# imdea-software/legosnark

Measured on AMD Instinct MI355X. Metric: alt_bn128 G1 MSM point-scalar pairs/s at n=2^20, higher is better.
Workload: dtype u32 limbs (254-bit Montgomery integers)

## Files before the change

### legosnark_amd/csrc/curves.h

```cpp
#pragma once
#include "ec.h"
#include "fp29.h"
#include "fp29x2.h"
#include "quad29.h"

namespace lsa {

struct CurveG1 {
    using Field = Fq;
    using Base = AffPacked;
    using Acc = XYZZ29;
    static constexpr bool GLV = true;
    static __device__ __forceinline__ Acc inf() { return Acc::inf(); }
    template <bool ENDO = true>
    static __device__ __forceinline__ Acc madd(const Acc &a, const Base &b, bool negate, bool endo) {
        return g1_madd_packed<ENDO>(a, b, negate, endo);
    }
    static constexpr bool HEAD = true;
    static __device__ __forceinline__ bool head_ok(const Base &b0, const Base &b1) { return !packed_is_inf(b0) && !packed_is_inf(b1); }
    template <bool ENDO = true>
    static __device__ __forceinline__ Acc madd_head(const Base &b0, bool neg0, bool endo0, const Base &b1, bool neg1, bool endo1) {
        return g1_madd_head<ENDO>(b0, neg0, endo0, b1, neg1, endo1);
    }
    static __device__ __forceinline__ Acc add(const Acc &a, const Acc &b) { return xyzz29_add(a, b); }
    static __device__ __forceinline__ Acc dbl(const Acc &a) { return xyzz29_dbl(a); }
    static __device__ __forceinline__ Jac<Fq> to_jac(const Acc &a) { return xyzz29_to_jac(a); }
    static __device__ __forceinline__ Acc from_jac(const Jac<Fq> &p) {
        if (p.Z.is_zero()) return Acc::inf();
        F29 z = F29::from_mont256(p.Z), zz = sqr(z);
        return {F29::from_mont256(p.X), F29::from_mont256(p.Y), zz, mul(zz, z)};
    }
    static __device__ __forceinline__ Base from_affine(const Aff<Fq> &a) {
        Base r;
        if (a.is_inf()) {
#pragma unroll
            for (int i = 0; i < 8; i++) { r.x[i] = 0; r.y[i] = 0; }
        } else {
            F29::from_mont256(a.x).canonical().pack256(r.x);
            F29::from_mont256(a.y).canonical().pack256(r.y);
        }
        return r;
    }
};
struct CurveG2 {
    using Field = Fq2;
    using Base = AffPackedG2;
    using Acc = XYZZ29x2;
    static constexpr bool GLV = false;
    static __device__ __forceinline__ Acc inf() { return Acc::inf(); }
    static constexpr bool HEAD = false;
    template <bool ENDO = true>
    static __device__ __forceinline__ Acc madd(const Acc &a, const Base &b, bool negate, bool ) {
        Aff29x2 q = unpack_affine(b);
        if (q.is_inf()) return a;
        if (negate) q.y = sub_k<1>(F29x2::zero(), q.y);
        return g2_madd(a, q);
    }
    static __device__ __forceinline__ Acc add(const Acc &a, const Acc &b) { return g2_add(a, b); }
    static __device__ __forceinline__ Acc dbl(const Acc &a) { return g2_dbl(a); }
    static __device__ __forceinline__ Jac<Fq2> to_jac(const Acc &a) { return g2_to_jac(a); }
    static __device__ __forceinline__ Acc from_jac(const Jac<Fq2> &p) {
        if (p.Z.is_zero()) return Acc::inf();
        F29x2 z = f29x2_from_mont256(p.Z), zz = sqr<2>(z);
        return {f29x2_from_mont256(p.X), f29x2_from_mont256(p.Y), zz, mul<2>(zz, z)};
    }
    static __device__ __forceinline__ Base from_affine(const Aff<Fq2> &a) { return pack_affine_g2(a); }
};
template <class F> struct CurveOf;
template <> struct CurveOf<Fq> { using type = CurveG1; };
template <> struct CurveOf<Fq2> { using type = CurveG2; };


}
```

### legosnark_amd/csrc/fp29.h

```cpp
#pragma once
#include "ec.h"

namespace lsa {

LSA_HD uint32_t lsa_mask(uint32_t m) {
#if defined(__HIP_DEVICE_COMPILE__)
    asm volatile("" : "+v"(m));
#endif
    return m;
}

struct F29 {
    static constexpr int W = 29;
    static constexpr uint32_t MASK = (1u << 29) - 1;
    static constexpr uint32_t PINV = 0x04866389u;
    static constexpr uint32_t PINV_POS = 0x1b799c77u;
    uint32_t l[9];

    static LSA_HD uint32_t p(int i) {
        constexpr uint32_t P29[9] = {0x187cfd47u, 0x010460b6u, 0x1c72a34fu, 0x02d522d0u, 0x1585d978u,
                                     0x02db40c0u, 0x00a6e141u, 0x0e5c2634u, 0x0030644eu};
        return P29[i];
    }
    static LSA_HD F29 from_limbs(const uint32_t (&c)[9]) {
        F29 r;
#pragma unroll
        for (int i = 0; i < 9; i++) r.l[i] = c[i];
        return r;
    }
    static LSA_HD F29 zero() {
        F29 r;
#pragma unroll
        for (int i = 0; i < 9; i++) r.l[i] = 0;
        return r;
    }
    static LSA_HD F29 one() {
        constexpr uint32_t C[9] = {0x157ccc21u, 0x141c2758u, 0x185230d3u, 0x014c0419u, 0x0aa36fb9u,
                                   0x1d4240ceu, 0x11d54c07u, 0x052ac7a8u, 0x000dc836u};
        return from_limbs(C);
    }
    LSA_HD bool limbs_zero() const {
        uint32_t o = 0;
#pragma unroll
        for (int i = 0; i < 9; i++) o |= l[i];
        return o == 0;
    }

    LSA_HD F29 norm() const {
        F29 r;
        int32_t c = 0;
#pragma unroll
        for (int i = 0; i < 8; i++) {
            int32_t v = (int32_t)l[i] + c;
            r.l[i] = (uint32_t)v & MASK;
            c = v >> 29;
        }
        r.l[8] = (uint32_t)((int32_t)l[8] + c);
        return r;
    }

    friend LSA_HD F29 add_lazy(const F29 &a, const F29 &b) {
        F29 r;
#pragma unroll
        for (int i = 0; i < 9; i++) r.l[i] = a.l[i] + b.l[i];
        return r;
    }
    template <int K>
    friend LSA_HD F29 sub_k(const F29 &a, const F29 &b);

    static LSA_HD F29 redc_cols(uint64_t (&col)[17]) {
        uint64_t carry = 0;
        F29 r;
#pragma unroll
        for (int k = 0; k < 9; k++) {
            uint64_t acc = col[k] + carry;
            const uint32_t m = ((uint32_t)acc * PINV) & MASK;
            acc += (uint64_t)m * p(0);
            carry = acc >> 29;
#pragma unroll
            for (int j = 1; j < 9; j++) col[k + j] += (uint64_t)m * p(j);
        }
#pragma unroll
        for (int k = 9; k < 17; k++) {
            const uint64_t acc = col[k] + carry;
            r.l[k - 9] = (uint32_t)acc & MASK;
            carry = acc >> 29;
        }
        r.l[8] = (uint32_t)carry;
        return r;
    }
    friend LSA_HD F29 mul(const F29 &a, const F29 &b) {
#if defined(LSA_FP29_COLS)
        {
            uint64_t col[17];
#pragma unroll
            for (int k = 0; k < 17; k++) col[k] = 0;
#pragma unroll
            for (int i = 0; i < 9; i++)
#pragma unroll
                for (int j = 0; j < 9; j++) col[i + j] += (uint64_t)a.l[i] * b.l[j];
            return redc_cols(col);
        }
#endif
        uint64_t acc = 0;
        uint32_t m[9];
        F29 r;
#pragma unroll
        for (int k = 0; k < 9; k++) {
#pragma unroll
            for (int i = 0; i <= k; i++) acc += (uint64_t)a.l[i] * b.l[k - i];
#pragma unroll
            for (int i = 0; i < k; i++) acc += (uint64_t)m[i] * p(k - i);
            m[k] = ((uint32_t)acc * PINV) & MASK;
            acc += (uint64_t)m[k] * p(0);
            acc >>= 29;
        }
#pragma unroll
        for (int k = 9; k < 17; k++) {
#pragma unroll
            for (int i = k - 8; i < 9; i++) acc += (uint64_t)a.l[i] * b.l[k - i];
#pragma unroll
            for (int i = k - 8; i < 9; i++) acc += (uint64_t)m[i] * p(k - i);
            r.l[k - 9] = (uint32_t)acc & MASK;
            acc >>= 29;
        }
        r.l[8] = (uint32_t)acc;
        return r;
    }
    friend LSA_HD F29 sqr(const F29 &a) {
        uint32_t d[9];
#pragma unroll
        for (int i = 0; i < 9; i++) d[i] = a.l[i] << 1;
#if defined(LSA_FP29_COLS)
        {
            uint64_t col[17];
#pragma unroll
            for (int k = 0; k < 17; k++) col[k] = 0;
#pragma unroll
            for (int i = 0; i < 9; i++) {
                col[2 * i] += (uint64_t)a.l[i] * a.l[i];
#pragma unroll
                for (int j = i + 1; j < 9; j++) col[i + j] += (uint64_t)a.l[i] * d[j];
            }
            return redc_cols(col);
        }
#endif
        uint64_t acc = 0;
        uint32_t m[9];
        F29 r;
#pragma unroll
        for (int k = 0; k < 17; k++) {
#pragma unroll
            for (int i = 0; i < 9; i++) {
// ... 88 lines not shown
                acc += (uint64_t)a1.l[i] * b1.l[k - i];
                acc += (uint64_t)a2.l[i] * b2.l[k - i];
                acc += (uint64_t)a3.l[i] * b3.l[k - i];
            }
#pragma unroll
            for (int i = k - 8; i < 9; i++) acc += (uint64_t)m[i] * p(k - i);
            r.l[k - 9] = (uint32_t)acc & MASK;
            acc >>= 29;
        }
        r.l[8] = (uint32_t)acc;
        return r;
    }
    friend LSA_HD F29 lin2(const F29 &u, int cu, const F29 &v, int cv, int K) {
        F29 r;
        int64_t c = 0;
#pragma unroll
        for (int i = 0; i < 9; i++) {
#if defined(__HIP_DEVICE_COMPILE__)
            int64_t t = c;
            asm("v_mad_i64_i32 %0, vcc, %1, %2, %0" : "+v"(t) : "v"(K), "v"((int32_t)p(i)) : "vcc");
            asm("v_mad_i64_i32 %0, vcc, %1, %2, %0" : "+v"(t) : "v"(cu), "v"((int32_t)u.l[i]) : "vcc");
            asm("v_mad_i64_i32 %0, vcc, %1, %2, %0" : "+v"(t) : "v"(cv), "v"((int32_t)v.l[i]) : "vcc");
#else
            const int64_t t = (int64_t)cu * (int64_t)u.l[i] + (int64_t)cv * (int64_t)v.l[i] + (int64_t)K * (int64_t)p(i) + c;
#endif
            if (i < 8) { r.l[i] = (uint32_t)t & MASK; c = t >> 29; }
            else r.l[i] = (uint32_t)t;
        }
        return r;
    }

    LSA_HD bool is_zero_mod_p() const {
        uint32_t k = (l[0] * PINV_POS) & MASK;
        if (k >= 16) return false;
        uint64_t c = 0;
        bool eq = true;
#pragma unroll
        for (int i = 0; i < 9; i++) {
            c += (uint64_t)k * p(i);
            uint32_t want = (i < 8) ? ((uint32_t)c & MASK) : (uint32_t)c;
            eq = eq && (want == l[i]);
            c >>= 29;
        }
        return eq;
    }

    LSA_HD F29 canonical() const {
        F29 t = *this;
#pragma unroll
        for (int s = 3; s >= 0; s--) {
            F29 d;
            int32_t c = 0;
            uint64_t pc = 0;
#pragma unroll
            for (int i = 0; i < 9; i++) {
                pc += (uint64_t)p(i) << s;
                uint32_t pl = (i < 8) ? ((uint32_t)pc & MASK) : (uint32_t)pc;
                pc >>= 29;
                int32_t v = (int32_t)t.l[i] - (int32_t)pl + c;
                if (i < 8) { d.l[i] = (uint32_t)v & MASK; c = v >> 29; }
                else d.l[i] = (uint32_t)v;
            }
            bool neg = ((int32_t)d.l[8]) < 0;
#pragma unroll
            for (int i = 0; i < 9; i++) t.l[i] = neg ? t.l[i] : d.l[i];
        }
        return t;
    }

    static LSA_HD F29 unpack256(const uint32_t w[8]) {
        F29 r;
#pragma unroll
        for (int i = 0; i < 9; i++) {
            const int bit = 29 * i, j = bit >> 5, s = bit & 31;
            uint64_t two = (uint64_t)w[j] | ((uint64_t)(j + 1 < 8 ? w[j + 1] : 0) << 32);
            r.l[i] = (uint32_t)(two >> s) & MASK;
        }
        return r;
    }
    LSA_HD void pack256(uint32_t w[8]) const {
#pragma unroll
        for (int j = 0; j < 8; j++) w[j] = 0;
#pragma unroll
        for (int i = 0; i < 9; i++) {
            const int bit = 29 * i, j = bit >> 5, s = bit & 31;
            uint64_t v = (uint64_t)l[i] << s;
            w[j] |= (uint32_t)v;
            if (j + 1 < 8) w[j + 1] |= (uint32_t)(v >> 32);
        }
    }
    static LSA_HD F29 from_mont256(const Fq &v) {
        constexpr uint32_t C[9] = {0x13349ca1u, 0x1a5d84a8u, 0x0a3e5cacu, 0x100249e0u, 0x12b951e8u,
                                   0x0e92d304u, 0x14cb95b3u, 0x041b9d3du, 0x00058003u};
        return mul(unpack256(v.l), from_limbs(C));
    }
    LSA_HD Fq to_mont256() const {
        constexpr uint32_t D[9] = {0x058f0d9du, 0x1aea1c6eu, 0x11c2cf74u, 0x11d651ebu, 0x1462c0a7u,
                                   0x11b7bc3cu, 0x1cbd99bau, 0x183340fbu, 0x000e0a77u};
        F29 t = mul(*this, from_limbs(D)).canonical();
        Fq r;
        t.pack256(r.l);
        return r;
    }
};

template <int K>
LSA_HD F29 sub_k(const F29 &a, const F29 &b) {
    F29 r;
    uint64_t pc = 0;
    int32_t c = 0;
#pragma unroll
    for (int i = 0; i < 9; i++) {
        pc += (uint64_t)F29::p(i) * (uint32_t)K;
        uint32_t kp = (i < 8) ? ((uint32_t)pc & F29::MASK) : (uint32_t)pc;
        pc >>= 29;
        int32_t v = (int32_t)a.l[i] + (int32_t)kp - (int32_t)b.l[i] + c;
        if (i < 8) { r.l[i] = (uint32_t)v & F29::MASK; c = v >> 29; }
        else r.l[i] = (uint32_t)v;
    }
    return r;
}

template <int K>
LSA_HD F29 sub_k_signed(const F29 &s, const F29 &b, uint32_t m) {
    F29 r;
    uint64_t pc = 0;
    const uint32_t m29 = m & F29::MASK;
    int32_t c = (int32_t)(m & 1u);
#pragma unroll
    for (int i = 0; i < 9; i++) {
        pc += (uint64_t)F29::p(i) * (uint32_t)K;
        uint32_t kp = (i < 8) ? ((uint32_t)pc & F29::MASK) : (uint32_t)pc;
        pc >>= 29;
        int32_t v = (int32_t)(s.l[i] ^ (i < 8 ? m29 : m)) + (int32_t)kp - (int32_t)b.l[i] + c;
        if (i < 8) { r.l[i] = (uint32_t)v & F29::MASK; c = v >> 29; }
        else r.l[i] = (uint32_t)v;
    }
    return r;
}

template <int K>
LSA_HD F29 sub_loose(const F29 &a, const F29 &b) {
    F29 r;
    uint64_t pc = 0;
#pragma unroll
    for (int i = 0; i < 9; i++) {
        pc += (uint64_t)F29::p(i) * (uint32_t)K;
        const uint32_t kp = (i < 8) ? ((uint32_t)pc & F29::MASK) : (uint32_t)pc;
        pc >>= 29;
        const uint32_t c = (i == 0) ? kp + (1u << 29) : (i < 8) ? kp + F29::MASK : kp - 1u;
        r.l[i] = a.l[i] + c - b.l[i];
    }
    return r;
}

struct Aff29 {
    F29 x, y;
    LSA_HD bool is_inf() const { return x.limbs_zero() && y.limbs_zero(); }
};
struct AffPacked {
    uint32_t x[8], y[8];
};
struct XYZZ29 {
    F29 X, Y, ZZ, ZZZ;
    LSA_HD bool is_inf() const { return ZZ.limbs_zero(); }
    static LSA_HD XYZZ29 inf() { return {F29::zero(), F29::zero(), F29::zero(), F29::zero()}; }
};

LSA_HD Aff29 unpack_affine(const AffPacked &q) { return {F29::unpack256(q.x), F29::unpack256(q.y)}; }

LSA_HD XYZZ29 xyzz29_dbl_affine(const Aff29 &b) {
    F29 U = add_lazy(b.y, b.y);
    F29 V = sqr(U);
    F29 W = mul(U, V);
    F29 S = mul(b.x, V);
    F29 xx = sqr(b.x);
    F29 M = add_lazy(add_lazy(xx, xx), xx).norm();
    F29 X3 = sub_k<4>(sqr(M), add_lazy(S, S));
    F29 Y3 = dot2(M, sub_k<8>(S, X3), W, sub_k<1>(F29::zero(), b.y));
    return {X3, Y3, V, W};
}

LSA_HD XYZZ29 xyzz29_dbl(const XYZZ29 &a) {
    if (a.is_inf()) return a;
    F29 U = add_lazy(a.Y, a.Y);
    F29 V = sqr(U);
    F29 W = mul(U, V);
    F29 S = mul(a.X, V);
    F29 xx = sqr(a.X);
    F29 M = add_lazy(add_lazy(xx, xx), xx).norm();
    F29 X3 = sub_k<4>(sqr(M), add_lazy(S, S));
    F29 Y3 = dot2(M, sub_k<8>(S, X3), W, sub_k<4>(F29::zero(), a.Y));
    return {X3, Y3, mul(V, a.ZZ), mul(W, a.ZZZ)};
}

LSA_HD XYZZ29 xyzz29_madd(const XYZZ29 &a, const Aff29 &b) {
    if (b.is_inf()) return a;
    if (a.is_inf()) return {b.x, b.y, F29::one(), F29::one()};
    F29 U2 = mul(b.x, a.ZZ);
    F29 S2 = mul(b.y, a.ZZZ);
    F29 Pd = sub_k<8>(U2, a.X);
    F29 R = sub_k<4>(S2, a.Y);
    if (Pd.is_zero_mod_p()) {
        if (R.is_zero_mod_p()) return xyzz29_dbl_affine(b);
        return XYZZ29::inf();
    }
    F29 PP = sqr(Pd);
    F29 PPP = mul(Pd, PP);
    F29 Q = mul(a.X, PP);
    F29 X3 = sub_k<6>(sqr(R), add_lazy(PPP, add_lazy(Q, Q)));
    F29 Y3 = dot2(R, sub_k<8>(Q, X3), sub_k<4>(F29::zero(), a.Y), PPP);
    return {X3, Y3, mul(a.ZZ, PP), mul(a.ZZZ, PPP)};
}

LSA_HD XYZZ29 xyzz29_madd_rare(const XYZZ29 &a, const Aff29 &b, uint32_t m, const F29 &R) {
    Aff29 q = b;
    if (m) q.y = sub_k<1>(F29::zero(), b.y);
    if (a.is_inf()) return {q.x, q.y, F29::one(), F29::one()};
    if (R.is_zero_mod_p()) return xyzz29_dbl_affine(q);
    return XYZZ29::inf();
}
LSA_HD XYZZ29 xyzz29_madd_signed(const XYZZ29 &a, const Aff29 &b, uint32_t m) {
    F29 U2 = mul(b.x, a.ZZ);
    F29 S2 = mul(b.y, a.ZZZ);
    F29 Pd = sub_k<8>(U2, a.X);
    F29 R = sub_k_signed<6>(S2, a.Y, m);
    if (Pd.is_zero_mod_p()) return xyzz29_madd_rare(a, b, m, R);
    F29 PP = sqr(Pd);
    F29 PPP = mul(Pd, PP);
    F29 Q = mul(a.X, PP);
    F29 X3 = sub_k<6>(sqr(R), add_lazy(PPP, add_lazy(Q, Q)));
    F29 Y3 = dot2(R, sub_loose<10>(Q, X3), sub_loose<6>(F29::zero(), a.Y), PPP);
    return {X3, Y3, mul(a.ZZ, PP), mul(a.ZZZ, PPP)};
}

LSA_HD XYZZ29 xyzz29_add_affine(const Aff29 &a, const Aff29 &b, uint32_t m) {
    F29 Pd = sub_k<2>(b.x, a.x);
    F29 R = sub_k_signed<2>(b.y, a.y, m);
    if (Pd.is_zero_mod_p()) {
        if (!R.is_zero_mod_p()) return XYZZ29::inf();
        Aff29 q = b;
        if (m) q.y = sub_k<1>(F29::zero(), b.y);
        return xyzz29_dbl_affine(q);
    }
    F29 PP = sqr(Pd);
    F29 PPP = mul(Pd, PP);
    F29 Q = mul(a.x, PP);
    F29 X3 = sub_k<6>(sqr(R), add_lazy(PPP, add_lazy(Q, Q)));
    F29 Y3 = dot2(R, sub_loose<10>(Q, X3), sub_loose<3>(F29::zero(), a.y), PPP);
    return {X3, Y3, PP, PPP};
}

LSA_HD XYZZ29 xyzz29_add(const XYZZ29 &a, const XYZZ29 &b) {
    if (b.is_inf()) return a;
    if (a.is_inf()) return b;
    F29 U1 = mul(a.X, b.ZZ);
    F29 U2 = mul(b.X, a.ZZ);
    F29 S1 = mul(a.Y, b.ZZZ);
    F29 S2 = mul(b.Y, a.ZZZ);
    F29 Pd = sub_k<2>(U2, U1);
    F29 R = sub_k<2>(S2, S1);
    if (Pd.is_zero_mod_p()) {
        if (R.is_zero_mod_p()) return xyzz29_dbl(a);
        return XYZZ29::inf();
    }
    F29 PP = sqr(Pd);
    F29 PPP = mul(Pd, PP);
    F29 Q = mul(U1, PP);
    F29 X3 = sub_k<6>(sqr(R), add_lazy(PPP, add_lazy(Q, Q)));
    F29 Y3 = dot2(R, sub_k<8>(Q, X3), sub_k<2>(F29::zero(), S1), PPP);
    return {X3, Y3, mul(mul(a.ZZ, b.ZZ), PP), mul(mul(a.ZZZ, b.ZZZ), PPP)};
}

LSA_HD bool packed_is_inf(const AffPacked &q) {
    if ((q.x[0] | q.y[0]) != 0) return false;
    uint32_t o = 0;
#pragma unroll
    for (int i = 1; i < 8; i++) o |= q.x[i] | q.y[i];
    return o == 0;
}
template <bool ENDO>
LSA_HD Aff29 g1_unpack_base(const AffPacked &b, bool endo) {
    Aff29 q = unpack_affine(b);
    if (ENDO && endo) {
        constexpr uint32_t BETA29[9] = {0x0a337995u, 0x158d1d23u, 0x189c9b98u, 0x12fa4e45u, 0x185faadcu,
                                        0x0176f16du, 0x0eed93bau, 0x14291140u, 0x000c0afeu};
        q.x = mul(q.x, F29::from_limbs(BETA29));
    }
    return q;
}
template <bool ENDO>
LSA_HD XYZZ29 g1_madd_packed(const XYZZ29 &a, const AffPacked &b, bool negate, bool endo) {
    if (packed_is_inf(b)) return a;
    return xyzz29_madd_signed(a, g1_unpack_base<ENDO>(b, endo), lsa_mask(negate ? ~0u : 0u));
}
template <bool ENDO>
LSA_HD XYZZ29 g1_madd_head(const AffPacked &b0, bool neg0, bool endo0, const AffPacked &b1, bool neg1, bool endo1) {
    Aff29 q0 = g1_unpack_base<ENDO>(b0, endo0);
    if (neg0) q0.y = sub_k<1>(F29::zero(), q0.y);
    return xyzz29_add_affine(q0, g1_unpack_base<ENDO>(b1, endo1), lsa_mask(neg1 ? ~0u : 0u));
}

LSA_HD XYZZ29 xyzz29_neg(const XYZZ29 &a) {
    if (a.is_inf()) return a;
    return {a.X, sub_k<4>(F29::zero(), a.Y), a.ZZ, a.ZZZ};
}

LSA_HD Jac<Fq> xyzz29_to_jac(const XYZZ29 &a) {
    if (a.is_inf()) return Jac<Fq>::inf();
    F29 Xj = mul(a.X, sqr(a.ZZ));
    F29 Yj = mul(a.Y, sqr(a.ZZZ));
    return {Xj.to_mont256(), Yj.to_mont256(), a.ZZZ.to_mont256()};
}

}
```

### legosnark_amd/csrc/msm.hip

```cpp
#include <hip/hip_runtime.h>
#include <stdint.h>
#include <stdio.h>
#include <stdlib.h>
#include <string.h>
#include <algorithm>
#include <type_traits>
#include <vector>

#include "curves.h"
#include "fp29x2l.h"
#include "fs29.h"
#include "glv.h"
#include "msm.h"
#include "msm_plan.h"

namespace lsa {


template <class F, int K>
__global__ __launch_bounds__(256) void k_normalize(const Jac<F> *__restrict__ in, Aff<F> *__restrict__ out, size_t n) {
    size_t t = (size_t)blockIdx.x * blockDim.x + threadIdx.x;
    size_t base = t * K;
    if (base >= n) return;
    F prod[K];
// ... 709 lines not shown
            perm[bin_start[bin] + lcnt[bin] + rank[j]] = g;
        }
    }
}

typedef uint32_t u32x4 __attribute__((ext_vector_type(4)));
template <class B> struct RawBase {
    static_assert(sizeof(B) % 16 == 0, "packed bases are whole 16-byte vectors");
    u32x4 q[sizeof(B) / 16];
};
template <class B>
__device__ __forceinline__ RawBase<B> load_base16(const B *__restrict__ p) {
    const u32x4 *src = reinterpret_cast<const u32x4 *>(p);
    RawBase<B> r;
#pragma unroll
    for (int i = 0; i < (int)(sizeof(B) / 16); i++) r.q[i] = src[i];
    return r;
}
template <class B>
__device__ __forceinline__ B packed_base(RawBase<B> r) {
    B b;
    uint32_t *dst = reinterpret_cast<uint32_t *>(&b);
#pragma unroll
    for (int i = 0; i < (int)(sizeof(B) / 16); i++) {
        asm("" : "+v"(r.q[i]));
        dst[4 * i] = r.q[i].x; dst[4 * i + 1] = r.q[i].y; dst[4 * i + 2] = r.q[i].z; dst[4 * i + 3] = r.q[i].w;
    }
    return b;
}
template <class C> struct RotatedLoads { static constexpr bool value = true; };
template <> struct RotatedLoads<CurveG2> { static constexpr bool value = false; };
template <class C, uint32_t ACC_SPLIT, bool ROTATED = RotatedLoads<C>::value>
__device__ __forceinline__ void accumulate_body(const typename C::Base *__restrict__ bases, const uint32_t *__restrict__ entries,
                                                const uint32_t *__restrict__ offs, const uint32_t *__restrict__ hist,
                                                const uint32_t *__restrict__ perm, const uint32_t *__restrict__ nperm,
                                                typename C::Acc *__restrict__ buckets) {
    uint32_t t = blockIdx.x * blockDim.x + threadIdx.x;
    if (t >= *nperm * ACC_SPLIT) return;
    const uint32_t g = perm[t / ACC_SPLIT], part = t % ACC_SPLIT;
    const uint32_t cnt = hist[g];
    const uint32_t *e = entries + offs[g];
    constexpr bool ENDO = ACC_SPLIT != 1;
    typename C::Acc acc = C::inf();
    if constexpr (!ROTATED) {
        if (part < cnt) {
            uint32_t v = e[part];
            typename C::Base cur = bases[v & 0x3fffffffu];
            static_assert(!C::HEAD || ROTATED, "the affine + affine head is written for the rotated loop only");
            for (uint32_t j = part; j < cnt; j += ACC_SPLIT) {
                uint32_t vn = v;
                typename C::Base nxt = cur;
                if (j + ACC_SPLIT < cnt) { vn = e[j + ACC_SPLIT]; nxt = bases[vn & 0x3fffffffu]; }
                acc = C::template madd<ENDO>(acc, cur, (v >> 31) != 0, ((v >> 30) & 1) != 0);
                v = vn;
                cur = nxt;
            }
        }
    } else if (part < cnt) {
        const uint32_t last = part + (cnt - 1 - part) / ACC_SPLIT * ACC_SPLIT;
        auto word = [&](uint32_t k) { return e[k < last ? k : last]; };
        auto base = [&](uint32_t w) { return load_base16(bases + (w & 0x3fffffffu)); };
        uint32_t j = part;
        uint32_t v = word(j), vn = word(j + ACC_SPLIT);
        RawBase<typename C::Base> cur;
        if constexpr (C::HEAD) {
            const uint32_t v2 = word(j + 2 * ACC_SPLIT), v3 = word(j + 3 * ACC_SPLIT);
            const RawBase<typename C::Base> r0 = base(v), r1 = base(vn), r2 = base(v2);
            const typename C::Base b0 = packed_base(r0), b1 = packed_base(r1);
            cur = r0;
            if (j + ACC_SPLIT < cnt && C::head_ok(b0, b1)) {
                acc = C::template madd_head<ENDO>(b0, (v >> 31) != 0, ((v >> 30) & 1) != 0, b1, (vn >> 31) != 0, ((vn >> 30) & 1) != 0);
                j += 2 * ACC_SPLIT;
                v = v2;
                vn = v3;
                cur = r2;
            }
        } else {
            cur = base(v);
        }
        for (; j < cnt; j += ACC_SPLIT) {
            const uint32_t vnn = word(j + 2 * ACC_SPLIT);
            const RawBase<typename C::Base> nxt = base(vn);
            acc = C::template madd<ENDO>(acc, packed_base(cur), (v >> 31) != 0, ((v >> 30) & 1) != 0);
            v = vn;
            vn = vnn;
            cur = nxt;
        }
    }
    buckets[(size_t)g * ACC_SPLIT + part] = acc;
}
template <class C, uint32_t ACC_SPLIT>
__global__ __launch_bounds__(256) void k_accumulate(const typename C::Base *__restrict__ bases, const uint32_t *__restrict__ entries,
                                                    const uint32_t *__restrict__ offs, const uint32_t *__restrict__ hist,
                                                    const uint32_t *__restrict__ perm, const uint32_t *__restrict__ nperm,
                                                    typename C::Acc *__restrict__ buckets) {
    accumulate_body<C, ACC_SPLIT>(bases, entries, offs, hist, perm, nperm, buckets);
}
__global__ __launch_bounds__(256) __attribute__((amdgpu_waves_per_eu(2, 2))) void k_accumulate_g2_occ2(
    const CurveG2::Base *__restrict__ bases, const uint32_t *__restrict__ entries, const uint32_t *__restrict__ offs,
    const uint32_t *__restrict__ hist, const uint32_t *__restrict__ perm, const uint32_t *__restrict__ nperm, CurveG2::Acc *__restrict__ buckets) {
    accumulate_body<CurveG2, 1u>(bases, entries, offs, hist, perm, nperm, buckets);
}

__global__ __launch_bounds__(256) void k_accumulate_g2_pair(const AffPackedG2 *__restrict__ bases, const uint32_t *__restrict__ entries,
                                                            const uint32_t *__restrict__ offs, const uint32_t *__restrict__ hist,
                                                            const uint32_t *__restrict__ perm, const uint32_t *__restrict__ nperm,
                                                            XYZZ29x2 *__restrict__ buckets) {
    const uint32_t t = blockIdx.x * blockDim.x + threadIdx.x, pr = t >> 1, part = t & 1;
    if (pr >= *nperm) return;
    const uint32_t g = perm[pr];
    const uint32_t cnt = hist[g];
    const uint32_t *e = entries + offs[g];
    struct Half { uint32_t x[8], y[8]; };
    auto fetch = [&](uint32_t v) {
        const AffPackedG2 &b = bases[v & 0x3fffffffu];
        Half h;
#pragma unroll
        for (int i = 0; i < 8; i++) { h.x[i] = b.w[part][i]; h.y[i] = b.w[2 + part][i]; }
        return h;
    };
    XyzzE<F29h> acc = XyzzE<F29h>::inf();
    uint32_t v = e[0];
    Half cur = fetch(v);
    for (uint32_t j = 0; j < cnt; j++) {
        uint32_t vn = v;
        Half nxt = cur;
        if (j + 1 < cnt) { vn = e[j + 1]; nxt = fetch(vn); }
        AffE<F29h> q = {{F29::unpack256(cur.x)}, {F29::unpack256(cur.y)}};
        if (!q.is_inf()) {
            if (v >> 31) q.y = sub_k<1>(F29h::zero(), q.y);
            acc = g2_madd(acc, q);
        }
        v = vn;
        cur = nxt;
    }
    F29 *o = reinterpret_cast<F29 *>(&buckets[g]);
    o[part] = acc.X.v;
    o[2 + part] = acc.Y.v;
    o[4 + part] = acc.ZZ.v;
    o[6 + part] = acc.ZZZ.v;
}

template <class A>
__device__ __forceinline__ A shfl_down_acc(const A &p, unsigned delta) {
    A r;
    constexpr int NW = sizeof(A) / 4;
    const uint32_t *src = reinterpret_cast<const uint32_t *>(&p);
    uint32_t *dst = reinterpret_cast<uint32_t *>(&r);
#pragma unroll
    for (int i = 0; i < NW; i++) dst[i] = __shfl_down(src[i], delta, 64);
    return r;
}

template <class C>
__device__ __forceinline__ typename C::Acc wave_sum(typename C::Acc v, unsigned lane) {
    for (unsigned d = 32; d >= 1; d >>= 1) {
        typename C::Acc t = shfl_down_acc(v, d);
        if (lane + d < 64) v = C::add(v, t);
    }
    return v;
}

__global__ __launch_bounds__(256) void k_heavy_plan(const uint32_t *__restrict__ hist, const uint32_t *__restrict__ heavy_list,
                                                    const uint32_t *__restrict__ heavy_count, uint32_t *__restrict__ chunk_off) {
    __shared__ uint32_t lds[4];
    __shared__ uint32_t s_chunk;
    const uint32_t nh = *heavy_count;
    uint32_t carry = 0;
    for (uint32_t base = 0; base < nh; base += 256) {
        uint32_t h = base + threadIdx.x;
        uint32_t tot;
        (void)block_exclusive_scan_256(h < nh ? hist[heavy_list[h]] : 0, lds, &tot);
        carry += tot;
    }
    if (threadIdx.x == 0) {
        uint32_t chunk = HEAVY_CHUNK;
        while (chunk < 4096u && carry / (2 * chunk) >= 2048u) chunk *= 2;
        s_chunk = chunk;
    }
    __syncthreads();
    const uint32_t chunk = s_chunk;
    carry = 0;
    for (uint32_t base = 0; base < nh; base += 256) {
        uint32_t h = base + threadIdx.x;
        uint32_t v = h < nh ? (hist[heavy_list[h]] + chunk - 1) / chunk : 0;
        uint32_t tot;
        uint32_t ex = block_exclusive_scan_256(v, lds, &tot);
        if (h < nh) chunk_off[h] = carry + ex;
        carry += tot;
    }
    if (threadIdx.x == 0) { chunk_off[nh] = carry; chunk_off[nh + 1] = chunk; }
}

template <class C>
__global__ __launch_bounds__(64) void k_accumulate_heavy(const typename C::Base *__restrict__ bases, const uint32_t *__restrict__ entries,
                                                         const uint32_t *__restrict__ offs, const uint32_t *__restrict__ hist,
                                                         const uint32_t *__restrict__ heavy_list, const uint32_t *__restrict__ heavy_count,
                                                         const uint32_t *__restrict__ chunk_off, typename C::Acc *__restrict__ partials) {
    const uint32_t nh = *heavy_count;
    if (nh == 0) return;
    const uint32_t total = chunk_off[nh], chunk = chunk_off[nh + 1];
    const unsigned lane = threadIdx.x;
    for (uint32_t v = blockIdx.x; v < total; v += gridDim.x) {
        uint32_t lo = 0, hi = nh;
        while (hi - lo > 1) { uint32_t mid = (lo + hi) >> 1; if (chunk_off[mid] <= v) lo = mid; else hi = mid; }
        const uint32_t g = heavy_list[lo];
        const uint32_t cnt = hist[g];
        const uint32_t start = (v - chunk_off[lo]) * chunk;
        const uint32_t end = start + chunk < cnt ? start + chunk : cnt;
        const uint32_t *e = entries + offs[g];
        typename C::Acc acc = C::inf();
        uint32_t j = start + lane;
        if constexpr (!RotatedLoads<C>::value) {
            for (; j < end; j += 64) {
                uint32_t w = e[j];
                acc = C::madd(acc, bases[w & 0x3fffffffu], (w >> 31) != 0, ((w >> 30) & 1) != 0);
            }
        } else if (j < end) {
            const uint32_t last = j + (end - 1 - j) / 64 * 64;
            auto word = [&](uint32_t k) { return e[k < last ? k : last]; };
            uint32_t w = word(j), wn = word(j + 64);
            RawBase<typename C::Base> cur = load_base16(bases + (w & 0x3fffffffu));
            for (; j < end; j += 64) {
                const uint32_t wnn = word(j + 128);
                const RawBase<typename C::Base> nxt = load_base16(bases + (wn & 0x3fffffffu));
                acc = C::madd(acc, packed_base(cur), (w >> 31) != 0, ((w >> 30) & 1) != 0);
                w = wn;
                wn = wnn;
                cur = nxt;
            }
        }
        acc = wave_sum<C>(acc, lane);
        if (lane == 0) partials[v] = acc;
    }
}

template <class C>
__global__ __launch_bounds__(64) void k_heavy_finish(const uint32_t *__restrict__ heavy_list, const uint32_t *__restrict__ heavy_count,
                                                     const uint32_t *__restrict__ chunk_off, const typename C::Acc *__restrict__ partials,
                                                     typename C::Acc *__restrict__ buckets, uint32_t split) {
    const uint32_t nh = *heavy_count;
    unsigned lane = threadIdx.x;
    for (uint32_t h = blockIdx.x; h < nh; h += gridDim.x) {
        typename C::Acc acc = C::inf();
        for (uint32_t v = chunk_off[h] + lane; v < chunk_off[h + 1]; v += 64) acc = C::add(acc, partials[v]);
        acc = wave_sum<C>(acc, lane);
        if (lane == 0) {
            buckets[(size_t)heavy_list[h] * split] = acc;
            for (uint32_t x = 1; x < split; x++) buckets[(size_t)heavy_list[h] * split + x] = C::inf();
        }
    }
}

template <class A>
__device__ __forceinline__ A select_acc(uint32_t mask, const A &a, const A &b) {
    A r;
    const uint32_t *pa = reinterpret_cast<const uint32_t *>(&a), *pb = reinterpret_cast<const uint32_t *>(&b);
    uint32_t *pr = reinterpret_cast<uint32_t *>(&r);
#pragma unroll
    for (int i = 0; i < (int)(sizeof(A) / 4); i++) pr[i] = (pa[i] & mask) | (pb[i] & ~mask);
    return r;
}
template <class A>
__device__ __forceinline__ void quadwave_weighted(A &acc, A &run, unsigned log_mult, unsigned lane) {
    const unsigned q = lane & 3, qi = lane >> 2;
    A s = A::inf();
#pragma unroll 1
    for (unsigned step = 0; step < 9; step++) {
        if (step == 4) {
            s = (qi == 0) ? A::inf() : run;
#pragma unroll 1
            for (unsigned i = 0; i < log_mult; i++) s = quad_dbl(s, q);
        }
        uint32_t m_run = step < 4 ? 0xffffffffu : 0u, m_s = step == 4 ? 0xffffffffu : 0u;
        asm volatile("" : "+v"(m_run), "+v"(m_s));
        const unsigned d = step < 4 ? (1u << step) : (step == 4 ? 0u : (8u >> (step - 5)));
        const A lhs = select_acc(m_run, run, acc);
        const A rhs = select_acc(m_s, s, shfl_down_acc(lhs, 4 * d));
        A r = lhs;
        if (qi + d < 16) r = quad_add(lhs, rhs, q);
        run = select_acc(m_run, r, run);
        acc = select_acc(m_run, acc, r);
    }
}

template <class C>
__global__ __launch_bounds__(64) void k_reduce1_lane(const typename C::Acc *__restrict__ buckets, uint32_t B, uint32_t L, uint32_t split,
                                                     typename C::Acc *__restrict__ out) {
    using A = typename C::Acc;
    const uint32_t t = blockIdx.x * 64 + threadIdx.x;
    if ((uint64_t)t * L >= B) return;
    A acc = A::inf(), run = A::inf();
    const A *bk = buckets + (size_t)t * L * split;
    const uint32_t per = split + 1;
#pragma unroll 1
    for (int i = (int)L - 1; i >= 0; i--) {
#pragma unroll 1
        for (uint32_t h = 0; h < per; h++) {
            uint32_t m = h < split ? 0xffffffffu : 0u;
            asm volatile("" : "+v"(m));
            A rhs = run;
            if (h < split) rhs = bk[(size_t)i * split + h];
            const A lhs = select_acc(m, run, acc);
            const A r = C::add(lhs, rhs);
            run = select_acc(m, r, run);
            acc = select_acc(m, acc, r);
        }
    }
    out[2 * (size_t)t] = acc;
    out[2 * (size_t)t + 1] = run;
}

template <class C>
__global__ __launch_bounds__(64) void k_reduce2_lane(const typename C::Acc *__restrict__ in, uint32_t m_in, uint32_t m_out, uint32_t log_mult,
                                                     typename C::Acc *__restrict__ out) {
    using A = typename C::Acc;
    const uint32_t t = blockIdx.x * 64 + threadIdx.x;
    if (t >= m_out) return;
    A acc = A::inf(), run = A::inf(), wsum = A::inf();
#pragma unroll 1
    for (int j = 15; j >= 0; j--) {
        const uint32_t idx = 16 * t + (uint32_t)j;
        const bool have = idx < m_in;
        const uint32_t trips = j ? 3u : 2u;
#pragma unroll 1
        for (uint32_t h = 0; h < trips; h++) {
            uint32_t m0 = h == 0 ? 0xffffffffu : 0u, m1 = h == 1 ? 0xffffffffu : 0u;
            asm volatile("" : "+v"(m0), "+v"(m1));
            A rhs = run;
            if (h < 2) rhs = have ? in[2 * (size_t)idx + h] : A::inf();
            const A lhs = select_acc(m0, acc, select_acc(m1, run, wsum));
            const A r = C::add(lhs, rhs);
            acc = select_acc(m0, r, acc);
            run = select_acc(m1, r, run);
            wsum = select_acc(~(m0 | m1), r, wsum);
        }
    }
#pragma unroll 1
    for (uint32_t i = 0; i < log_mult; i++) wsum = C::dbl(wsum);
    out[2 * (size_t)t] = C::add(acc, wsum);
    out[2 * (size_t)t + 1] = run;
}

template <class C>
__global__ __launch_bounds__(64) void k_reduce1(const typename C::Acc *__restrict__ buckets, uint32_t B, uint32_t L, uint32_t logL,
                                                uint32_t waves_per_window, uint32_t split, typename C::Acc *__restrict__ wave_out) {
    using A = typename C::Acc;
    uint32_t wave = blockIdx.x;
    uint32_t k = wave / waves_per_window, w = wave % waves_per_window;
    const unsigned lane = threadIdx.x, q = lane & 3;
    uint32_t t = w * 16 + (lane >> 2);
    A acc = A::inf(), run = A::inf();
    if ((uint64_t)t * L < B) {
        const A *bk = buckets + ((size_t)k * B + (size_t)t * L) * split;
        const uint32_t per = split + 1;
#pragma unroll 1
        for (int i = (int)L - 1; i >= 0; i--) {
#pragma unroll 1
            for (uint32_t h = 0; h < per; h++) {
                uint32_t m = h < split ? 0xffffffffu : 0u;
                asm volatile("" : "+v"(m));
                A rhs = run;
                if (h < split) rhs = bk[(size_t)i * split + h];
                const A lhs = select_acc(m, run, acc);
                const A r = quad_add(lhs, rhs, q);
                run = select_acc(m, r, run);
                acc = select_acc(m, acc, r);
            }
        }
    }
    quadwave_weighted(acc, run, logL, lane);
    if (lane == 0) {
        wave_out[2 * (size_t)wave] = acc;
        wave_out[2 * (size_t)wave + 1] = run;
    }
}

template <class C>
__global__ __launch_bounds__(64) void k_reduce2(const typename C::Acc *__restrict__ in, uint32_t m_in, uint32_t m_out, uint32_t log_mult,
                                                typename C::Acc *__restrict__ out) {
    using A = typename C::Acc;
    const uint32_t k = blockIdx.x / m_out, w = blockIdx.x % m_out;
    const unsigned lane = threadIdx.x;
    const uint32_t j = w * 16 + (lane >> 2);
    A acc = A::inf(), run = A::inf();
    if (j < m_in) {
        acc = in[2 * ((size_t)k * m_in + j)];
        run = in[2 * ((size_t)k * m_in + j) + 1];
    }
    quadwave_weighted(acc, run, log_mult, lane);
    if (lane == 0) {
        out[2 * ((size_t)k * m_out + w)] = acc;
        out[2 * ((size_t)k * m_out + w) + 1] = run;
    }
}

template <class A>
__device__ __forceinline__ void pin_vgpr(A &a) {
    uint32_t *w = reinterpret_cast<uint32_t *>(&a);
#pragma unroll
    for (int i = 0; i < (int)(sizeof(A) / 4); i++) asm volatile("" : "+v"(w[i]));
}

template <class A, class J>
__device__ __forceinline__ void fold_quad_body(const A *__restrict__ window_sums, unsigned nwin, unsigned c, J *__restrict__ out) {
    if (blockIdx.x != 0) return;
    const unsigned q = threadIdx.x & 3;
    A r = window_sums[2 * (nwin - 1)];
    pin_vgpr(r);
    for (int k = (int)nwin - 2; k >= 0; k--) {
        for (unsigned i = 0; i < c; i++) r = quad_dbl(r, q);
        A w = window_sums[2 * k];
        pin_vgpr(w);
        r = quad_add(r, w, q);
    }
    J res;
    if constexpr (std::is_same<A, XYZZ29>::value) res = xyzz29_to_jac(r);
    else res = g2_to_jac(r);
    pin_vgpr(res);
    if (threadIdx.x == 0) *out = res;
}
__global__ __launch_bounds__(64) void k_fold_quad(const XYZZ29 *__restrict__ window_sums, unsigned nwin, unsigned c, Jac<Fq> *__restrict__ out) {
    fold_quad_body(window_sums, nwin, c, out);
}
__global__ __launch_bounds__(64) void k_fold_quad_g2(const XYZZ29x2 *__restrict__ window_sums, unsigned nwin, unsigned c, Jac<Fq2> *__restrict__ out) {
    fold_quad_body(window_sums, nwin, c, out);
}

template <class A, class J>
__device__ __forceinline__ void emit_body(const A *__restrict__ window_sums, J *__restrict__ out) {
    if (threadIdx.x != 0) return;
    A r = window_sums[2 * (size_t)blockIdx.x];
    if constexpr (std::is_same<A, XYZZ29>::value) out[blockIdx.x] = xyzz29_to_jac(r);
    else out[blockIdx.x] = g2_to_jac(r);
}
__global__ __launch_bounds__(64) void k_emit_g1(const XYZZ29 *__restrict__ window_sums, Jac<Fq> *__restrict__ out) { emit_body(window_sums, out); }
__global__ __launch_bounds__(64) void k_emit_g2(const XYZZ29x2 *__restrict__ window_sums, Jac<Fq2> *__restrict__ out) { emit_body(window_sums, out); }

template <class A>
__device__ __forceinline__ A bits_quad_tree(A a, unsigned lane, unsigned first_d) {
    const unsigned sub = lane & 3, qd = lane >> 2;
#pragma unroll 1
    for (unsigned d = first_d; d >= 1; d >>= 1) {
        A o = shfl_down_acc(a, 4 * d);
        if (qd + d >= 16) o = A::inf();
        a = quad_add(a, o, sub);
    }
    return a;
}
template <class C>
__global__ __launch_bounds__(512) void k_reduce_bits_a(const typename C::Acc *__restrict__ pairs, uint32_t m, uint32_t nbits, uint32_t G,
                                                       typename C::Acc *__restrict__ part) {
    using A = typename C::Acc;
    constexpr uint32_t AW = sizeof(A) / 4;
    __shared__ uint32_t wave_sum[8][AW];
    const uint32_t bit = blockIdx.x, g = blockIdx.y;
    const unsigned tid = threadIdx.x, lane = tid & 63, wv = tid >> 6, sub = lane & 3, qd = lane >> 2;
    A a = A::inf();
#pragma unroll 1
    for (uint32_t j = 0; j < 4; j++) {
        const uint32_t t = g * 512 + wv * 64 + qd + 16 * j;
        A o = A::inf();
        if (t < m) {
            if (bit == nbits) o = pairs[2 * (size_t)t];
            else if ((t >> bit) & 1u) o = pairs[2 * (size_t)t + 1];
        }
        a = quad_add(a, o, sub);
    }
    a = bits_quad_tree(a, lane, 8);
    if (lane == 0) {
        const uint32_t *src = reinterpret_cast<const uint32_t *>(&a);
#pragma unroll
        for (uint32_t w = 0; w < AW; w++) wave_sum[wv][w] = src[w];
    }
    __syncthreads();
    if (wv != 0) return;
    a = A::inf();
    if (qd < 8) a = *reinterpret_cast<const A *>(&wave_sum[qd][0]);
    a = bits_quad_tree(a, lane, 4);
    if (lane == 0) part[bit * G + g] = a;
}
template <class C>
__global__ __launch_bounds__(64) void k_reduce_bits_b(const typename C::Acc *__restrict__ part, uint32_t nbits, uint32_t G, uint32_t lm,
                                                      typename C::Acc *__restrict__ weighted) {
    using A = typename C::Acc;
    const uint32_t bit = blockIdx.x;
    const unsigned lane = threadIdx.x, sub = lane & 3, qd = lane >> 2;
    A a = A::inf();
    if (qd < G) a = part[bit * G + qd];
    a = bits_quad_tree(a, lane, 8);
    const uint32_t dbl = bit == nbits ? 0u : lm + bit;
#pragma unroll 1
    for (uint32_t i = 0; i < dbl; i++) a = quad_dbl(a, sub);
// ... 667 lines not shown
```

Before: 785.1 million.

## Interleave pairs of independent Montgomery multiplications in G1 point addition

Adds mul2/sqr2 helpers that compute two independent 9-limb Montgomery products in one column-interleaved chain, with scheduling barriers that keep the two MAC streams alternating. The G1 mixed-add, affine-add and a new paired XYZZ add use these helpers, and the paired add is enabled in the heavy-bucket and reduce1 tail kernels. The goal is more instruction-level parallelism by hiding the latency of the dependent 64-bit multiply-accumulate chain. In exchange it uses more live registers, which may lower occupancy, and the sched_barrier calls may block other compiler scheduling.

```diff
diff --git a/legosnark_amd/csrc/curves.h b/legosnark_amd/csrc/curves.h
--- a/legosnark_amd/csrc/curves.h
+++ b/legosnark_amd/csrc/curves.h
@@ -22,7 +22,11 @@
     static __device__ __forceinline__ Acc madd_head(const Base &b0, bool neg0, bool endo0, const Base &b1, bool neg1, bool endo1) {
         return g1_madd_head<ENDO>(b0, neg0, endo0, b1, neg1, endo1);
     }
-    static __device__ __forceinline__ Acc add(const Acc &a, const Acc &b) { return xyzz29_add(a, b); }
+    template <bool PAIRED = false>
+    static __device__ __forceinline__ Acc add(const Acc &a, const Acc &b) {
+        if constexpr (PAIRED) return xyzz29_add_paired(a, b);
+        else return xyzz29_add(a, b);
+    }
     static __device__ __forceinline__ Acc dbl(const Acc &a) { return xyzz29_dbl(a); }
     static __device__ __forceinline__ Jac<Fq> to_jac(const Acc &a) { return xyzz29_to_jac(a); }
     static __device__ __forceinline__ Acc from_jac(const Jac<Fq> &p) {
@@ -56,6 +60,7 @@
         if (negate) q.y = sub_k<1>(F29x2::zero(), q.y);
         return g2_madd(a, q);
     }
+    template <bool PAIRED = false>
     static __device__ __forceinline__ Acc add(const Acc &a, const Acc &b) { return g2_add(a, b); }
     static __device__ __forceinline__ Acc dbl(const Acc &a) { return g2_dbl(a); }
     static __device__ __forceinline__ Jac<Fq2> to_jac(const Acc &a) { return g2_to_jac(a); }
diff --git a/legosnark_amd/csrc/fp29.h b/legosnark_amd/csrc/fp29.h
--- a/legosnark_amd/csrc/fp29.h
+++ b/legosnark_amd/csrc/fp29.h
@@ -1,4 +1,5 @@
 #pragma once
+#include <utility>
 #include "ec.h"
 
 namespace lsa {
@@ -393,6 +394,105 @@
         r.l[i] = a.l[i] + c - b.l[i];
     }
     return r;
+}
+
+struct MacPaired {
+    static LSA_HD void mac(uint64_t &acc, uint32_t a, uint32_t b) {
+        acc += (uint64_t)a * b;
+#if defined(__HIP_DEVICE_COMPILE__)
+        asm volatile("" : "+v"(acc));
+        __builtin_amdgcn_sched_barrier(0);
+#endif
+    }
+};
+struct MulTerms {
+    const F29 &a, &b;
+    static constexpr int count(int k) { return k < 9 ? k + 1 : 17 - k; }
+    template <class Mac>
+    LSA_HD void term(uint64_t &acc, int k, int s) const {
+        const int i = (k < 9 ? 0 : k - 8) + s;
+        Mac::mac(acc, a.l[i], b.l[k - i]);
+    }
+};
+struct SqrTerms {
+    const F29 &a;
+    const uint32_t (&d)[9];
+    static constexpr int lo(int k) { return k < 9 ? 0 : k - 8; }
+    static constexpr int cross(int k) { return (k + 1) / 2 - lo(k); }
+    static constexpr int count(int k) { return cross(k) + ((k & 1) == 0 ? 1 : 0); }
+    template <class Mac>
+    LSA_HD void term(uint64_t &acc, int k, int s) const {
+        if (s < cross(k)) Mac::mac(acc, a.l[lo(k) + s], d[k - lo(k) - s]);
+        else Mac::mac(acc, a.l[k / 2], a.l[k / 2]);
+    }
+};
+struct F29Pair {
+    F29 a, b;
+};
+template <class Mac, class T0, class T1>
+struct F29Chain2 {
+    uint64_t acc0 = 0, acc1 = 0;
+    uint32_t m0[9], m1[9];
+    F29Pair r;
+    template <int K>
+    LSA_HD void column(const T0 &t0, const T1 &t1) {
+        constexpr int N0 = T0::count(K), N1 = T1::count(K), N = N0 > N1 ? N0 : N1;
+#pragma unroll
+        for (int s = 0; s < N; s++) {
+            if (s < N0) t0.template term<Mac>(acc0, K, s);
+            if (s < N1) t1.template term<Mac>(acc1, K, s);
+        }
+#pragma unroll
+        for (int i = (K < 9 ? 0 : K - 8); i < (K < 9 ? K : 9); i++) {
+            Mac::mac(acc0, m0[i], F29::p(K - i));
+            Mac::mac(acc1, m1[i], F29::p(K - i));
+        }
+        if constexpr (K < 9) {
+            m0[K] = ((uint32_t)acc0 * F29::PINV) & F29::MASK;
+            m1[K] = ((uint32_t)acc1 * F29::PINV) & F29::MASK;
+            Mac::mac(acc0, m0[K], F29::p(0));
+            Mac::mac(acc1, m1[K], F29::p(0));
+        } else {
+            r.a.l[K - 9] = (uint32_t)acc0 & F29::MASK;
+            r.b.l[K - 9] = (uint32_t)acc1 & F29::MASK;
+        }
+        acc0 >>= 29;
+        acc1 >>= 29;
+    }
+    template <int... K>
+    LSA_HD void columns(const T0 &t0, const T1 &t1, std::integer_sequence<int, K...>) {
+        (column<K>(t0, t1), ...);
+    }
+};
+template <class Mac, class T0, class T1>
+LSA_HD F29Pair f29_chain2(const T0 &t0, const T1 &t1) {
+    F29Chain2<Mac, T0, T1> c;
+    c.columns(t0, t1, std::make_integer_sequence<int, 17>{});
+    c.r.a.l[8] = (uint32_t)c.acc0;
+    c.r.b.l[8] = (uint32_t)c.acc1;
+    return c.r;
+}
+LSA_HD void f29_doubled(const F29 &a, uint32_t (&d)[9]) {
+#pragma unroll
+    for (int i = 0; i < 9; i++) d[i] = a.l[i] << 1;
+}
+
+LSA_HD F29Pair mul2(const F29 &a0, const F29 &b0, const F29 &a1, const F29 &b1) {
+#if defined(__HIP_DEVICE_COMPILE__)
+    return f29_chain2<MacPaired>(MulTerms{a0, b0}, MulTerms{a1, b1});
+#else
+    return {mul(a0, b0), mul(a1, b1)};
+#endif
+}
+LSA_HD F29Pair sqr2(const F29 &a0, const F29 &a1) {
+#if defined(__HIP_DEVICE_COMPILE__)
+    uint32_t d0[9], d1[9];
+    f29_doubled(a0, d0);
+    f29_doubled(a1, d1);
+    return f29_chain2<MacPaired>(SqrTerms{a0, d0}, SqrTerms{a1, d1});
+#else
+    return {sqr(a0), sqr(a1)};
+#endif
 }
 
 struct Aff29 {
@@ -462,17 +562,16 @@
     return XYZZ29::inf();
 }
 LSA_HD XYZZ29 xyzz29_madd_signed(const XYZZ29 &a, const Aff29 &b, uint32_t m) {
-    F29 U2 = mul(b.x, a.ZZ);
-    F29 S2 = mul(b.y, a.ZZZ);
-    F29 Pd = sub_k<8>(U2, a.X);
-    F29 R = sub_k_signed<6>(S2, a.Y, m);
+    const F29Pair us = mul2(b.x, a.ZZ, b.y, a.ZZZ);
+    F29 Pd = sub_k<8>(us.a, a.X);
+    F29 R = sub_k_signed<6>(us.b, a.Y, m);
     if (Pd.is_zero_mod_p()) return xyzz29_madd_rare(a, b, m, R);
-    F29 PP = sqr(Pd);
-    F29 PPP = mul(Pd, PP);
-    F29 Q = mul(a.X, PP);
-    F29 X3 = sub_k<6>(sqr(R), add_lazy(PPP, add_lazy(Q, Q)));
-    F29 Y3 = dot2(R, sub_loose<10>(Q, X3), sub_loose<6>(F29::zero(), a.Y), PPP);
-    return {X3, Y3, mul(a.ZZ, PP), mul(a.ZZZ, PPP)};
+    const F29Pair sq = sqr2(Pd, R);
+    const F29Pair pq = mul2(Pd, sq.a, a.X, sq.a);
+    F29 X3 = sub_k<6>(sq.b, add_lazy(pq.a, add_lazy(pq.b, pq.b)));
+    F29 Y3 = dot2(R, sub_loose<10>(pq.b, X3), sub_loose<6>(F29::zero(), a.Y), pq.a);
+    const F29Pair zz = mul2(a.ZZ, sq.a, a.ZZZ, pq.a);
+    return {X3, Y3, zz.a, zz.b};
 }
 
 LSA_HD XYZZ29 xyzz29_add_affine(const Aff29 &a, const Aff29 &b, uint32_t m) {
@@ -484,12 +583,11 @@
         if (m) q.y = sub_k<1>(F29::zero(), b.y);
         return xyzz29_dbl_affine(q);
     }
-    F29 PP = sqr(Pd);
-    F29 PPP = mul(Pd, PP);
-    F29 Q = mul(a.x, PP);
-    F29 X3 = sub_k<6>(sqr(R), add_lazy(PPP, add_lazy(Q, Q)));
-    F29 Y3 = dot2(R, sub_loose<10>(Q, X3), sub_loose<3>(F29::zero(), a.y), PPP);
-    return {X3, Y3, PP, PPP};
+    const F29Pair sq = sqr2(Pd, R);
+    const F29Pair pq = mul2(Pd, sq.a, a.x, sq.a);
+    F29 X3 = sub_k<6>(sq.b, add_lazy(pq.a, add_lazy(pq.b, pq.b)));
+    F29 Y3 = dot2(R, sub_loose<10>(pq.b, X3), sub_loose<3>(F29::zero(), a.y), pq.a);
+    return {X3, Y3, sq.a, pq.a};
 }
 
 LSA_HD XYZZ29 xyzz29_add(const XYZZ29 &a, const XYZZ29 &b) {
@@ -512,6 +610,25 @@
     F29 Y3 = dot2(R, sub_k<8>(Q, X3), sub_k<2>(F29::zero(), S1), PPP);
     return {X3, Y3, mul(mul(a.ZZ, b.ZZ), PP), mul(mul(a.ZZZ, b.ZZZ), PPP)};
 }
+LSA_HD XYZZ29 xyzz29_add_paired(const XYZZ29 &a, const XYZZ29 &b) {
+    if (b.is_inf()) return a;
+    if (a.is_inf()) return b;
+    const F29Pair u = mul2(a.X, b.ZZ, b.X, a.ZZ);
+    const F29Pair v = mul2(a.Y, b.ZZZ, b.Y, a.ZZZ);
+    F29 Pd = sub_k<2>(u.b, u.a);
+    F29 R = sub_k<2>(v.b, v.a);
+    if (Pd.is_zero_mod_p()) {
+        if (R.is_zero_mod_p()) return xyzz29_dbl(a);
+        return XYZZ29::inf();
+    }
+    const F29Pair sq = sqr2(Pd, R);
+    const F29Pair pq = mul2(Pd, sq.a, u.a, sq.a);
+    F29 X3 = sub_k<6>(sq.b, add_lazy(pq.a, add_lazy(pq.b, pq.b)));
+    F29 Y3 = dot2(R, sub_k<8>(pq.b, X3), sub_k<2>(F29::zero(), v.a), pq.a);
+    const F29Pair z = mul2(a.ZZ, b.ZZ, a.ZZZ, b.ZZZ);
+    const F29Pair zz = mul2(z.a, sq.a, z.b, pq.a);
+    return {X3, Y3, zz.a, zz.b};
+}
 
 LSA_HD bool packed_is_inf(const AffPacked &q) {
     if ((q.x[0] | q.y[0]) != 0) return false;
diff --git a/legosnark_amd/csrc/msm.hip b/legosnark_amd/csrc/msm.hip
--- a/legosnark_amd/csrc/msm.hip
+++ b/legosnark_amd/csrc/msm.hip
@@ -885,11 +885,16 @@
     return r;
 }
 
-template <class C>
+enum TailKernel { TAIL_HEAVY, TAIL_REDUCE1_LANE, TAIL_REDUCE2_LANE };
+template <class C, TailKernel K> struct PairedAdd { static constexpr bool value = false; };
+template <> struct PairedAdd<CurveG1, TAIL_HEAVY> { static constexpr bool value = true; };
+template <> struct PairedAdd<CurveG1, TAIL_REDUCE1_LANE> { static constexpr bool value = true; };
+
+template <class C, bool PAIRED = false>
 __device__ __forceinline__ typename C::Acc wave_sum(typename C::Acc v, unsigned lane) {
     for (unsigned d = 32; d >= 1; d >>= 1) {
         typename C::Acc t = shfl_down_acc(v, d);
-        if (lane + d < 64) v = C::add(v, t);
+        if (lane + d < 64) v = C::template add<PAIRED>(v, t);
     }
     return v;
 }
@@ -963,7 +968,7 @@
                 cur = nxt;
             }
         }
-        acc = wave_sum<C>(acc, lane);
+        acc = wave_sum<C, PairedAdd<C, TAIL_HEAVY>::value>(acc, lane);
         if (lane == 0) partials[v] = acc;
     }
 }
@@ -1035,7 +1040,7 @@
             A rhs = run;
             if (h < split) rhs = bk[(size_t)i * split + h];
             const A lhs = select_acc(m, run, acc);
-            const A r = C::add(lhs, rhs);
+            const A r = C::template add<PairedAdd<C, TAIL_REDUCE1_LANE>::value>(lhs, rhs);
             run = select_acc(m, r, run);
             acc = select_acc(m, acc, r);
         }
@@ -1063,7 +1068,7 @@
             A rhs = run;
             if (h < 2) rhs = have ? in[2 * (size_t)idx + h] : A::inf();
             const A lhs = select_acc(m0, acc, select_acc(m1, run, wsum));
-            const A r = C::add(lhs, rhs);
+            const A r = C::template add<PairedAdd<C, TAIL_REDUCE2_LANE>::value>(lhs, rhs);
             acc = select_acc(m0, r, acc);
             run = select_acc(m1, r, run);
             wsum = select_acc(~(m0 | m1), r, wsum);
@@ -1071,7 +1076,7 @@
     }
 #pragma unroll 1
     for (uint32_t i = 0; i < log_mult; i++) wsum = C::dbl(wsum);
-    out[2 * (size_t)t] = C::add(acc, wsum);
+    out[2 * (size_t)t] = C::template add<PairedAdd<C, TAIL_REDUCE2_LANE>::value>(acc, wsum);
     out[2 * (size_t)t + 1] = run;
 }
 
```

Result: faster. 834.2 million (median of 6 runs) (+6.3%).
